# craftsangjae/instance-segmentation-road-project

Measured on AMD Instinct MI355X. Metric: images/sec at 1024x1024 (MaskLab inference hot path, full forward), higher is better.
Workload: dtype f32; 1 GPU; resnext50_full_b8_1024; per_gpu_batch=8, global_batch=8, height=1024, width=1024, parallelism=dp1, hipgraph=False, inputs=resident in HBM, weights=random init (cls logits x8 so NMS / mask head run at full load)

## Files before the change

### include/masklab_hip.h

```cpp
#ifndef MASKLAB_HIP_H
#define MASKLAB_HIP_H

#include <stdint.h>

#ifdef __cplusplus
extern "C" {
#endif

#define ML_OK 0
#define ML_E_BADARG (-1)
#define ML_E_LAUNCH (-2)
#define ML_E_NOGPU  (-3)

enum { ML_ACT_NONE = 0, ML_ACT_RELU = 1, ML_ACT_RELU6 = 2, ML_ACT_SIGMOID = 3 };
enum { ML_MATH_F32 = 0, ML_MATH_F16 = 1, ML_MATH_F16S = 2, ML_MATH_F32X3 = 3 };

#define ML_ABI_VERSION 7
int ml_version(void);
const char *ml_last_error(void);
int ml_device_check(void);

typedef struct ml_conv2d_desc {
    const float *in;
    const float *wgt;
    const float *bias;
    const float *residual;
    float *out;
    int32_t B, H, W;
    int32_t in_cstride, in_coff;
    int32_t span;
    int32_t span_pad;
    int32_t cpp_shift;
    int32_t Ho, Wo;
    int32_t KH, KW, stride, dil, pad_t, pad_l;
    int32_t cout;
    int32_t n_pad;
    int32_t out_cstride, out_coff;
    int32_t res_cstride, res_coff;
    int32_t act;
    int32_t group_cin_step;
    int32_t shuffle2x2;
    int32_t tile;
    int32_t math;
    int32_t out_f16;
    int64_t out_bstride;
    const int32_t *live;
    int32_t live_period;
    int32_t reserved1;
    double *gn_partials;
} ml_conv2d_desc;

int ml_conv2d_f32(const ml_conv2d_desc *d, void *stream);

#define ML_CONV_MAX_PROBLEMS 12
int64_t ml_conv2d_workspace_bytes(void);
int ml_conv2d_multi_f32(const ml_conv2d_desc *descs, int32_t n, void *workspace, int64_t workspace_bytes,
                        void *stream);
int ml_conv2d_ntile(int32_t cout, int32_t tile);
int ml_conv2d_launch_ntile(const ml_conv2d_desc *descs, int32_t n, int32_t has_workspace);
int ml_conv2d_launch_mtile(const ml_conv2d_desc *descs, int32_t n, int32_t has_workspace);
int ml_conv2d_uses_pipe(const ml_conv2d_desc *d);
int ml_conv2d_launch_splits(const ml_conv2d_desc *descs, int32_t n, int64_t workspace_bytes, int32_t *splits);
int ml_conv2d_wino_eligible(const ml_conv2d_desc *d);
int64_t ml_conv2d_gn_min_launch_tiles(void);

int ml_gconv3x3_f32(const float *in, const float *wgt, const float *bias, float *out,
                    int32_t B, int32_t H, int32_t W, int32_t C, int32_t c, int32_t Ho, int32_t Wo,
                    int32_t stride, int32_t pad_t, int32_t pad_l, int32_t act, void *stream);

int ml_gconv3x3_f16(const void *in, const float *wgt, const float *bias, void *out,
                    int32_t B, int32_t H, int32_t W, int32_t C, int32_t c, int32_t Ho, int32_t Wo,
                    int32_t stride, int32_t pad_t, int32_t pad_l, int32_t act, void *stream);

int ml_maxpool3x3s2_f16(const void *in, void *out, int32_t B, int32_t H, int32_t W, int32_t C,
                        int32_t Ho, int32_t Wo, int32_t pad_t, int32_t pad_l, void *stream);
int ml_subsample2_f16(const void *in, void *out, int32_t B, int32_t H, int32_t W, int32_t C, void *stream);
int ml_cast_f16_to_f32(const void *in, float *out, int64_t n, void *stream);
int ml_cast_f32_to_f16(const float *in, void *out, int64_t n, void *stream);
int ml_resize_bilinear_ac_f16(const void *in, const void *add, void *out,
                              int32_t B, int32_t H, int32_t W, int32_t C, int32_t in_cstride, int32_t in_coff,
                              int32_t Ho, int32_t Wo, int32_t add_cstride, int32_t add_coff,
                              int32_t out_cstride, int32_t out_coff, void *stream);
int ml_dwconv3x3_f16(const void *in, const float *wgt, const float *bias, void *out,
                     int32_t B, int32_t H, int32_t W, int32_t C, int32_t in_cstride, int32_t in_coff,
                     int32_t out_cstride, int32_t out_coff, int32_t Ho, int32_t Wo,
                     int32_t stride, int32_t dil, int32_t pad_t, int32_t pad_l, int32_t act, void *stream);
int ml_global_mean_f16(const void *in, void *out, int32_t B, int32_t HW, int32_t C, void *stream);

int ml_stem7x7s2_pool_f16(const float *image, const void *wgt_h, const float *bias, void *out, int32_t B, int32_t H,
                          int32_t W, int32_t Hp, int32_t Wp, void *stream);
int ml_stem7x7s2_pool_f32(const float *image, const float *wgt, const float *bias, float *out, int32_t B, int32_t H,
                          int32_t W, int32_t Hp, int32_t Wp, void *stream);
int ml_stem7x7s2_pool_x3(const float *image, const void *wgt_x3, const float *bias, float *out, int32_t B, int32_t H,
                         int32_t W, int32_t Hp, int32_t Wp, void *stream);

typedef struct ml_deconv_out_problem {
    const float *x, *wd, *bd, *wo_table, *bo;
    float *out;
    int64_t M;
    int32_t hw, w, rois_per_image, reserved0;
    int64_t out_image_stride, out_base;
    const int32_t *live;
} ml_deconv_out_problem;
int ml_deconv2x2_out1x1_f32(const ml_deconv_out_problem *probs, int32_t nprob, int32_t K, int32_t c_mid, int32_t ncls,
                            int32_t cp, int32_t act_mid, int32_t act_out, void *stream);
int ml_deconv2x2_out1x1_f16(const ml_deconv_out_problem *probs, int32_t nprob, int32_t K, int32_t c_mid, int32_t ncls,
                            int32_t cp, int32_t act_mid, int32_t act_out, void *stream);

int ml_dwconv3x3_f32(const float *in, const float *wgt, const float *bias, float *out,
                     int32_t B, int32_t H, int32_t W, int32_t C,
                     int32_t in_cstride, int32_t in_coff, int32_t out_cstride, int32_t out_coff,
                     int32_t Ho, int32_t Wo, int32_t stride, int32_t dil,
                     int32_t pad_t, int32_t pad_l, int32_t act, void *stream);

int ml_maxpool3x3s2_f32(const float *in, float *out, int32_t B, int32_t H, int32_t W, int32_t C,
                        int32_t Ho, int32_t Wo, int32_t pad_t, int32_t pad_l, void *stream);

int ml_preprocess_f32(const void *in, int32_t is_u8, float *out, int64_t npix, int32_t out_c,
                      int32_t flip, const float *mean, const float *div, const float *shift,
                      void *stream);

int64_t ml_groupnorm_workspace_bytes(int32_t N, int32_t G);
int ml_groupnorm_chunk_f32(const float *x, float *y, const float *gamma, const float *beta,
                           int32_t N, int64_t HWC, int32_t C, int32_t G, float eps, int32_t relu,
                           int32_t out_cstride, int32_t out_coff,
                           void *workspace, void *stream);
int ml_groupnorm_chunk_f16(const void *x, void *y, const float *gamma, const float *beta,
                           int32_t N, int64_t HWC, int32_t C, int32_t G, float eps, int32_t relu,
                           int32_t out_cstride, int32_t out_coff, void *workspace, void *stream);

typedef struct ml_gn_desc {
    const float *x;
    float *y;
    const float *gamma, *beta;
    int64_t HWC;
    int32_t N, C, G, relu;
    int32_t out_cstride, out_coff;
    float eps;
    int32_t dtype;
    const int32_t *live;
    int32_t live_period, reserved;
    const double *partials;
    int32_t n_partials, reserved2;
} ml_gn_desc;
#define ML_GN_MAX_PROBLEMS 8
int ml_groupnorm_multi_f32(const ml_gn_desc *descs, int32_t n, void *workspace, int64_t workspace_bytes, void *stream);
// ... 237 lines not shown
```

### instance-segmentation-road-project_amd/csrc/conv_wino.hip

```cpp
#include "common.h"

namespace {

constexpr int WMAXP = ML_CONV_MAX_PROBLEMS;
constexpr int WT = 64;
constexpr int WN = 64;
constexpr int WK = 8;
constexpr int WCHUNK = WK * 32 * 16;
constexpr int WSTEP = 4 * 32 * 16;
constexpr int NSLOT_P = 3;
constexpr int SLOT_P = WT * 16 * 8;
constexpr int NSLOT_W = 4;
constexpr int SLOT_W = 2 * WSTEP;
constexpr int RING_W = NSLOT_P * SLOT_P;
constexpr int LDS_BYTES = (RING_W + NSLOT_W * SLOT_W) * 4;
static_assert(LDS_BYTES == 160 * 1024, "the two rings fill the CU's LDS");
#ifndef WINO_EXP
#define WINO_EXP 0
#endif
constexpr unsigned OOB = 0x80000000u;
constexpr long long SPAN_MAX = 0x7fffff00ll;

struct WProblem {
    ml_conv2d_desc d;
// ... 13 lines not shown
#endif
}

__device__ __forceinline__ void bt_d_b_op(int k, const float d[16], float t[16], float v[16]) {
    if (k < 16) {
        const int j = k >> 2;
        switch (k & 3) {
            case 0: t[0 * 4 + j] = d[0 * 4 + j] - d[2 * 4 + j]; break;
            case 1: t[1 * 4 + j] = d[1 * 4 + j] + d[2 * 4 + j]; break;
            case 2: t[2 * 4 + j] = d[2 * 4 + j] - d[1 * 4 + j]; break;
            default: t[3 * 4 + j] = d[1 * 4 + j] - d[3 * 4 + j]; break;
        }
    } else {
        const int i = (k - 16) >> 2;
        switch (k & 3) {
            case 0: v[i * 4 + 0] = t[i * 4 + 0] - t[i * 4 + 2]; break;
            case 1: v[i * 4 + 1] = t[i * 4 + 1] + t[i * 4 + 2]; break;
            case 2: v[i * 4 + 2] = t[i * 4 + 2] - t[i * 4 + 1]; break;
            default: v[i * 4 + 3] = t[i * 4 + 1] - t[i * 4 + 3]; break;
        }
    }
}

__global__ void __launch_bounds__(512, 1) conv_wino_kernel(const WArgs args) {
    extern __shared__ __align__(16) float lds[];

    int pi = 0;
    while (pi + 1 < args.n && (int)blockIdx.x >= args.start[pi + 1]) ++pi;
    const WProblem &P = args.p[pi];
    const ml_conv2d_desc &p = P.d;
    const int b = (int)blockIdx.x - args.start[pi];
    const int g = b / (8 * P.NB), rr = b - g * 8 * P.NB;
    const int nt2 = rr >> 3;
    const int mt = g * 8 + (rr & 7);
    if (mt >= P.MB) return;
    if (p.live) {
        const int lv = max(1, *p.live), tpi0 = P.TH * P.TW;
        const int b0 = mt * WT / tpi0, b1 = min(mt * WT + WT, P.T) - 1;
        bool any = false;
        for (int bi = b0; bi <= b1 / tpi0 && !any; ++bi) any = bi % p.live_period < lv;
        if (!any) return;
    }

    const int tid = threadIdx.x, lane = tid & 63;
    const int wave = __builtin_amdgcn_readfirstlane(tid >> 6);
    const int tg = wave & 3, h = wave >> 2;
    const int r = lane & 15, kq = lane >> 4;
    const int tpi = P.TH * P.TW;

    const int gt0 = mt * WT;
    long long base_pix;
    {
        const int bi = gt0 / tpi, rem = gt0 - bi * tpi, ty = rem / P.TW;
        base_pix = ((long long)bi * p.H + max(2 * ty - 1, 0)) * p.W;
    }
    const size_t cstride = (size_t)p.in_cstride;
    const float *pin = p.in + p.in_coff + (size_t)base_pix * cstride;
    int voff_p[4];
    {
        const int rt = (lane >> 1) & 15;
        const int quad = (lane & 1) ^ ((rt >> 2) & 1);
        const int gt = gt0 + (wave >> 1) * 16 + rt;
        int bi = 0, ty = 0, tx = 0;
        if (gt < P.T) {
            bi = gt / tpi;
            const int rem = gt - bi * tpi;
            ty = rem / P.TW;
            tx = rem - ty * P.TW;
        }
#pragma unroll
        for (int i = 0; i < 4; ++i) {
            const int px = 8 * (wave & 1) + 2 * i + (lane >> 5);
            const int y = 2 * ty - 1 + (px >> 2), x = 2 * tx - 1 + (px & 3);
            voff_p[i] = (int)OOB;
            if (gt < P.T && y >= 0 && y < p.H && x >= 0 && x < p.W)
                voff_p[i] = (int)((((long long)bi * p.H + y) * p.W + x - base_pix) * (long long)cstride * 4) + quad * 16;
        }
    }
    const int voff_w = ((wave & 3) * 512 + r * 16 + kq * 4) * 4;
    const float *wsrc = p.wgt + (size_t)(2 * nt2 + (wave >> 2)) * P.nchunks * WCHUNK;
    float *dst_p = lds + (wave >> 1) * 2048 + (wave & 1) * 1024;
    float *dst_w = lds + RING_W + (wave >> 2) * WSTEP + (wave & 3) * 512;
    const int nch = P.nchunks, nsteps = 2 * P.nchunks;

    auto rsrc_p = [&](int j) __attribute__((always_inline)) {
        const bool real = j < nch && !(WINO_EXP & 1);
        return __builtin_amdgcn_make_buffer_rsrc((void *)(pin + j * 8), 0, real ? (int)OOB : 0, 0x00020000);
    };
    auto rsrc_w = [&](int s) __attribute__((always_inline)) {
        const bool real = s < nsteps && !(WINO_EXP & 2);
        return __builtin_amdgcn_make_buffer_rsrc((void *)(wsrc + (size_t)s * WSTEP), 0, real ? WSTEP * 4 : 0, 0x00020000);
    };

    f32x4 acc[2][16];
#pragma unroll
    for (int t = 0; t < 2; ++t)
#pragma unroll
        for (int q = 0; q < 16; ++q) acc[t][q] = f32x4{0.f, 0.f, 0.f, 0.f};

    const float *pa_lane0 = lds + tg * 2048 + r * 8 + 4 * ((r >> 2) & 1) + kq;
    const float *pa_lane1 = lds + tg * 2048 + r * 8 + 4 * (((r >> 2) & 1) ^ 1) + kq;
    const float *pb_lane = lds + RING_W + h * WSTEP + kq * 512 + r * 4;
    struct Ops {
        float d[16], t[16], v[16];
        f32x4 b[2][4];
    };
    auto read_ops = [&](const float *pa, const float *pb, Ops &o) __attribute__((always_inline)) {
#pragma unroll
        for (int t = 0; t < 2; ++t)
#pragma unroll
            for (int pq = 0; pq < 4; ++pq) o.b[t][pq] = *reinterpret_cast<const f32x4 *>(pb + t * 256 + pq * 64);
#pragma unroll
        for (int px = 0; px < 16; ++px) o.d[px] = pa[px * 128];
    };

    auto step = [&](const Ops &cur, Ops &nxt, const float *pa, const float *pb, const int ndma, auto dma) __attribute__((always_inline)) {
#if WINO_EXP == 4
#pragma unroll
        for (int q = 0; q < ndma; ++q) dma(q);
        __builtin_amdgcn_sched_barrier(0);
#endif
#pragma unroll
        for (int m = 0; m < 32; ++m) {
            const int t = m >> 4, pq = (m >> 2) & 3, e = m & 3;
            acc[t][4 * pq + e] =
                __builtin_amdgcn_mfma_f32_16x16x4f32(cur.v[4 * pq + e], cur.b[t][pq][e], acc[t][4 * pq + e], 0, 0, 0);
            if (m == 3) {
                __builtin_amdgcn_sched_barrier(0);
                read_ops(pa, pb, nxt);
                __builtin_amdgcn_sched_barrier(0);
            }
#if WINO_EXP != 4
            if (m % 6 == 5 && m / 6 < ndma) {
                __builtin_amdgcn_sched_barrier(0);
                dma(m / 6);
                __builtin_amdgcn_sched_barrier(0);
            }
#endif
            if (m >= 16) {
                bt_d_b_op(2 * (m - 16), nxt.d, nxt.t, nxt.v);
                bt_d_b_op(2 * (m - 16) + 1, nxt.d, nxt.t, nxt.v);
                __builtin_amdgcn_sched_barrier(0);
            }
        }
    };

    {
        const __amdgpu_buffer_rsrc_t rp0 = rsrc_p(0), rp1 = rsrc_p(1), rw0 = rsrc_w(0), rw1 = rsrc_w(1), rw2 = rsrc_w(2);
#pragma unroll
        for (int i = 0; i < 4; ++i) dma16(rp0, dst_p + i * 256, voff_p[i]);
        dma16(rw0, dst_w, voff_w);
        dma16(rw0, dst_w + 256, voff_w + 1024);
#pragma unroll
        for (int i = 0; i < 4; ++i) dma16(rp1, dst_p + SLOT_P + i * 256, voff_p[i]);
        dma16(rw1, dst_w + SLOT_W, voff_w);
        dma16(rw1, dst_w + SLOT_W + 256, voff_w + 1024);
        dma16(rw2, dst_w + 2 * SLOT_W, voff_w);
        dma16(rw2, dst_w + 2 * SLOT_W + 256, voff_w + 1024);
    }
    Ops oa, ob;
    asm volatile("s_waitcnt vmcnt(8)" ::: "memory");
    __builtin_amdgcn_s_barrier();
    read_ops(pa_lane0, pb_lane, oa);
#pragma unroll
    for (int k = 0; k < 32; ++k) bt_d_b_op(k, oa.d, oa.t, oa.v);

    int ps0 = 0, ps1 = SLOT_P, ps2 = 2 * SLOT_P;
    for (int j = 0; j < nch; ++j) {
        const int w0 = (2 * j) & 3;
        const int wa = ((w0 ^ 2) + 1) * SLOT_W, wb = w0 * SLOT_W;
        asm volatile("s_waitcnt vmcnt(0) lgkmcnt(0)" ::: "memory");
        __builtin_amdgcn_s_barrier();
        const __amdgpu_buffer_rsrc_t rp = rsrc_p(j + 2), rwa = rsrc_w(2 * j + 3), rwb = rsrc_w(2 * j + 4);
        auto dma = [&](int q) __attribute__((always_inline)) {
            if (q < 4) dma16(rp, dst_p + ps2 + q * 256, voff_p[q]);
            else if (q < 6) dma16(rwa, dst_w + wa + (q - 4) * 256, voff_w + (q - 4) * 1024);
            else dma16(rwb, dst_w + wb + (q - 6) * 256, voff_w + (q - 6) * 1024);
        };
        step(oa, ob, pa_lane1 + ps0, pb_lane + (w0 + 1) * SLOT_W, 5, dma);
        step(ob, oa, pa_lane0 + ps1, pb_lane + (w0 ^ 2) * SLOT_W, 3, [&](int q) __attribute__((always_inline)) { dma(q + 5); });
        const int ps = ps0;
        ps0 = ps1;
        ps1 = ps2;
        ps2 = ps;
    }
    asm volatile("s_waitcnt vmcnt(0)" ::: "memory");

    const int nt = 2 * nt2 + h;
    const bool gn = p.gn_partials != nullptr;
    double gs[2] = {0.0, 0.0}, gq[2] = {0.0, 0.0};
    long long f0 = 0;
    if (gn) {
        const int bi = gt0 / tpi, rem = gt0 - bi * tpi, ty = rem / P.TW, tx = rem - ty * P.TW;
        f0 = ((long long)(bi * p.Ho + 2 * ty) * p.Wo + 2 * tx) >> 7;
    }
    const float lo = 0.f, hi = (p.act == ML_ACT_RELU6) ? 6.f : 3.402823466e38f;
    const bool clampv = p.act == ML_ACT_RELU || p.act == ML_ACT_RELU6;
#pragma unroll
    for (int i = 0; i < 4; ++i) {
        const int gt = gt0 + tg * 16 + kq * 4 + i;
        if (gt >= P.T) continue;
        const int bi = gt / tpi, rem = gt - bi * tpi;
        const int ty = rem / P.TW, tx = rem - ty * P.TW;
        const int oy = 2 * ty, ox = 2 * tx;
        const bool y1 = oy + 1 < p.Ho, x1 = ox + 1 < p.Wo;
        const size_t img = p.out_bstride ? (size_t)bi * (size_t)p.out_bstride : (size_t)bi * p.Ho * p.Wo * p.out_cstride;
        const size_t pix0 = (size_t)oy * p.Wo + ox;
#pragma unroll
        for (int t = 0; t < 2; ++t) {
            const int n = nt * 32 + 16 * t + r;
            if (n >= p.cout) continue;
            float m[16];
#pragma unroll
            for (int q = 0; q < 16; ++q) m[q] = acc[t][q][i];
            float u[8];
#pragma unroll
            for (int j = 0; j < 4; ++j) {
                u[j] = m[0 * 4 + j] + m[1 * 4 + j] + m[2 * 4 + j];
                u[4 + j] = m[1 * 4 + j] - m[2 * 4 + j] - m[3 * 4 + j];
            }
            float yv[4];
#pragma unroll
            for (int a = 0; a < 2; ++a) {
                yv[2 * a] = u[4 * a + 0] + u[4 * a + 1] + u[4 * a + 2];
                yv[2 * a + 1] = u[4 * a + 1] - u[4 * a + 2] - u[4 * a + 3];
            }
            const float bv = p.bias ? p.bias[n] : 0.f;
            float *o = p.out + img + p.out_coff + n;
#pragma unroll
            for (int a = 0; a < 2; ++a)
#pragma unroll
                for (int c2 = 0; c2 < 2; ++c2) {
                    if ((a && !y1) || (c2 && !x1)) continue;
                    float val = yv[2 * a + c2] + bv;
                    if (clampv) val = __builtin_amdgcn_fmed3f(val, lo, hi);
                    else if (p.act != ML_ACT_NONE) val = ml_apply_act(val, p.act);
                    o[(pix0 + (size_t)a * p.Wo + c2) * p.out_cstride] = val;
                    if (gn) {
                        const long long m_flat = ((long long)(bi * p.Ho + oy + a) * p.Wo + ox + c2);
                        const int f = (m_flat >> 7) != f0;
                        gs[f] += (double)val;
                        gq[f] += (double)val * (double)val;
                    }
                }
        }
    }
    if (gn) {
        double *lds_gn = reinterpret_cast<double *>(lds);
        __syncthreads();
#pragma unroll
        for (int o = 32; o > 0; o >>= 1) {
#pragma unroll
            for (int f = 0; f < 2; ++f) {
                gs[f] += __shfl_down(gs[f], o, 64);
                gq[f] += __shfl_down(gq[f], o, 64);
            }
        }
        if (lane == 0) {
            lds_gn[wave * 4 + 0] = gs[0]; lds_gn[wave * 4 + 1] = gq[0];
            lds_gn[wave * 4 + 2] = gs[1]; lds_gn[wave * 4 + 3] = gq[1];
        }
        __syncthreads();
        if (tid < 4) {
            const int hh = tid >> 1, ff = tid & 1;
            const int gt1 = gt0 + WT - 1;
            const int bi = gt1 / tpi, rem = gt1 - bi * tpi, ty = rem / P.TW, tx = rem - ty * P.TW;
            const long long f1 = ((long long)(bi * p.Ho + 2 * ty + 1) * p.Wo + 2 * tx + 1) >> 7;
            const long long ft = ff ? f1 : f0;
            const int slot = 2 * nt2 + hh;
            double s = 0.0, q = 0.0;
            for (int w = 0; w < 4; ++w) { s += lds_gn[(hh * 4 + w) * 4 + 2 * ff]; q += lds_gn[(hh * 4 + w) * 4 + 2 * ff + 1]; }
            p.gn_partials[2 * (ft * 4 + slot)] = s;
            p.gn_partials[2 * (ft * 4 + slot) + 1] = q;
        }
    }
}

}

extern "C" int ml_conv2d_wino_eligible(const ml_conv2d_desc *d) {
    if (!d) return 0;
    return d->math == ML_MATH_F32 && d->KH == 3 && d->KW == 3 && d->stride == 1 && d->dil == 1 && d->pad_t == 1 &&
           d->pad_l == 1 && d->Ho == d->H && d->Wo == d->W && d->cpp_shift == 30 && d->group_cin_step == 0 &&
           !d->shuffle2x2 && !d->residual && !d->out_f16 && d->span % 32 == 0 && d->span_pad == d->span &&
           d->cout <= 128 && d->n_pad == 128;
}

int ml_conv2d_wino_gn_ok(const ml_conv2d_desc &d) {
    if (d.Ho % 2 || d.Wo % 2 || d.cout != 128 || d.out_bstride || d.act == ML_ACT_SIGMOID) return 0;
    const long long TH = d.Ho / 2, TW = d.Wo / 2;
    return (64 % TW == 0 || TW % 64 == 0) && (TH * TW) % 64 == 0;
}

int ml_conv2d_wino_launch(const ml_conv2d_desc *descs, int n, hipStream_t s) {
    ML_REQUIRE(n >= 1 && n <= WMAXP, "conv2d (winograd): need 1..%d problems", WMAXP);
    WArgs args;
    args.n = n;
    long long start = 0;
    for (int i = 0; i < n; ++i) {
        const ml_conv2d_desc &d = descs[i];
        ML_REQUIRE(ml_conv2d_wino_eligible(&d),
                   "conv2d: tile = 6 (Winograd F(2x2,3x3)) needs ML_MATH_F32, a 3x3 stride-1 undilated 'same' conv, no "
                   "groups / shuffle / residual / half output, span %% 32 == 0 and n_pad == 128");
        ML_REQUIRE(((d.in_cstride | d.in_coff) & 3) == 0 && ml_aligned16(d.in) && ml_aligned16(d.wgt),
                   "conv2d (winograd): 16-byte aligned input channels and weights");
        if (d.gn_partials)
            ML_REQUIRE(ml_conv2d_wino_gn_ok(d) && !d.live, "conv2d (winograd): gn_partials needs even Ho / Wo, Wo / 2 dividing or a "
                                                "multiple of 64, (Ho / 2) (Wo / 2) %% 64 == 0, cout = 128, dense output");
        WProblem &P = args.p[i];
        P.d = d;
        P.TH = (d.Ho + 1) / 2;
        P.TW = (d.Wo + 1) / 2;
        const long long T = (long long)d.B * P.TH * P.TW;
        ML_REQUIRE(T < (1ll << 30), "conv2d (winograd): too many tiles");
        P.T = (int)T;
        P.MB = (int)((T + WT - 1) / WT);
        P.NB = d.n_pad / WN;
        P.nchunks = d.span_pad / WK;
        const long long span = (2ll * (WT / P.TW + 2) + 2) * d.W * d.in_cstride * 4;
        ML_REQUIRE(span <= SPAN_MAX, "conv2d (winograd): a block's input rows exceed 2 GiB (W x in_cstride too large)");
        args.start[i] = (int)start;
        start += (long long)(P.MB + 7) / 8 * 8 * P.NB;
        ML_REQUIRE(start < (1ll << 31), "conv2d (winograd): grid too large");
    }
    args.start[n] = (int)start;
    long long tiles128 = 0;
    bool any_gn = false;
    for (int i = 0; i < n; ++i) {
        tiles128 += ((long long)descs[i].B * descs[i].Ho * descs[i].Wo + 127) / 128 * (descs[i].n_pad / 128);
        any_gn = any_gn || descs[i].gn_partials != nullptr;
    }
    ML_REQUIRE(!any_gn || tiles128 >= ml_conv2d_gn_min_launch_tiles(),
               "conv2d (winograd): gn_partials needs a launch of ml_conv2d_gn_min_launch_tiles() tiles of 128 x 128");
    static std::atomic<unsigned long long> lds_ok{0};
    if (int rc = ml_ensure_dynamic_lds(reinterpret_cast<const void *>(conv_wino_kernel), LDS_BYTES, lds_ok, "conv2d (winograd)"))
        return rc;
    hipLaunchKernelGGL(conv_wino_kernel, dim3((unsigned)start), dim3(512), LDS_BYTES, s, args);
    ML_CHECK_LAUNCH("conv2d (winograd)");
    return ML_OK;
}
```

### instance-segmentation-road-project_amd/masklab_hip/_lib.py

```python
import ctypes as C
import os

_HERE = os.path.dirname(os.path.abspath(__file__))
LIB_PATH = os.path.join(_HERE, "libmasklab_hip.so")

ABI_VERSION = 7
ACT_NONE, ACT_RELU, ACT_RELU6, ACT_SIGMOID = 0, 1, 2, 3
ACT_BY_NAME = {None: ACT_NONE, "linear": ACT_NONE, "relu": ACT_RELU, "relu6": ACT_RELU6,
               "sigmoid": ACT_SIGMOID}


class ConvDesc(C.Structure):
    _fields_ = [
        ("in_", C.c_void_p), ("wgt", C.c_void_p), ("bias", C.c_void_p),
        ("residual", C.c_void_p), ("out", C.c_void_p),
        ("B", C.c_int32), ("H", C.c_int32), ("W", C.c_int32),
        ("in_cstride", C.c_int32), ("in_coff", C.c_int32),
        ("span", C.c_int32), ("span_pad", C.c_int32), ("cpp_shift", C.c_int32),
        ("Ho", C.c_int32), ("Wo", C.c_int32),
        ("KH", C.c_int32), ("KW", C.c_int32), ("stride", C.c_int32), ("dil", C.c_int32),
        ("pad_t", C.c_int32), ("pad_l", C.c_int32),
        ("cout", C.c_int32), ("n_pad", C.c_int32),
        ("out_cstride", C.c_int32), ("out_coff", C.c_int32),
        ("res_cstride", C.c_int32), ("res_coff", C.c_int32),
        ("act", C.c_int32), ("group_cin_step", C.c_int32), ("shuffle2x2", C.c_int32),
        ("tile", C.c_int32), ("math", C.c_int32), ("out_f16", C.c_int32),
        ("out_bstride", C.c_int64),
        ("live", C.c_void_p), ("live_period", C.c_int32), ("reserved1", C.c_int32),
        ("gn_partials", C.c_void_p),
    ]


class GnDesc(C.Structure):
    _fields_ = [("x", C.c_void_p), ("y", C.c_void_p), ("gamma", C.c_void_p), ("beta", C.c_void_p),
                ("HWC", C.c_int64), ("N", C.c_int32), ("C", C.c_int32), ("G", C.c_int32), ("relu", C.c_int32),
                ("out_cstride", C.c_int32), ("out_coff", C.c_int32), ("eps", C.c_float), ("dtype", C.c_int32),
                ("live", C.c_void_p), ("live_period", C.c_int32), ("reserved", C.c_int32),
                ("partials", C.c_void_p), ("n_partials", C.c_int32), ("reserved2", C.c_int32)]


class DeconvOutProblem(C.Structure):
    _fields_ = [("x", C.c_void_p), ("wd", C.c_void_p), ("bd", C.c_void_p), ("wo_table", C.c_void_p),
                ("bo", C.c_void_p), ("out", C.c_void_p), ("M", C.c_int64), ("hw", C.c_int32), ("w", C.c_int32),
                ("rois_per_image", C.c_int32), ("reserved0", C.c_int32), ("out_image_stride", C.c_int64),
                ("out_base", C.c_int64), ("live", C.c_void_p)]


class SeDesc(C.Structure):
    _fields_ = [("x", C.c_void_p), ("out", C.c_void_p), ("w1", C.c_void_p), ("w2", C.c_void_p),
                ("B", C.c_int32), ("HW", C.c_int32), ("C", C.c_int32), ("Hd", C.c_int32),
                ("live", C.c_void_p), ("live_period", C.c_int32), ("reserved", C.c_int32), ("ws_offset", C.c_int64)]


class SeResidualDesc(C.Structure):
    _fields_ = [("x", C.c_void_p), ("shortcut", C.c_void_p), ("w1", C.c_void_p), ("b1", C.c_void_p),
                ("w2", C.c_void_p), ("b2", C.c_void_p), ("scale", C.c_void_p), ("shift", C.c_void_p),
                ("out_act", C.c_void_p), ("out_y", C.c_void_p),
                ("B", C.c_int32), ("HW", C.c_int32), ("C", C.c_int32), ("Hd", C.c_int32),
                ("mode", C.c_int32), ("reserved", C.c_int32)]


class SeBottleneckDesc(C.Structure):
    _fields_ = [("c3", C.c_void_p), ("residual", C.c_void_p), ("w1", C.c_void_p), ("b1", C.c_void_p),
                ("w2", C.c_void_p), ("b2", C.c_void_p), ("out", C.c_void_p),
                ("B", C.c_int32), ("HW", C.c_int32), ("C", C.c_int32), ("Hd", C.c_int32)]


SE_RES_GATE, SE_RES_BN_RELU = 0, 1
GN_MAX_PROBLEMS = 8
SE_MAX_PROBLEMS = 8
DECONV_OUT_MAX_PROBLEMS = 4
_i32, _i64, _f32, _vp = C.c_int32, C.c_int64, C.c_float, C.c_void_p

SIGNATURES = {
    "ml_version": (C.c_int, []),
    "ml_last_error": (C.c_char_p, []),
    "ml_device_check": (C.c_int, []),
    "ml_conv2d_f32": (C.c_int, [C.POINTER(ConvDesc), _vp]),
    "ml_conv2d_ntile": (C.c_int, [_i32, _i32]),
    "ml_conv2d_uses_pipe": (C.c_int, [C.POINTER(ConvDesc)]),
    "ml_conv2d_launch_ntile": (C.c_int, [C.POINTER(ConvDesc), _i32, _i32]),
    "ml_conv2d_launch_mtile": (C.c_int, [C.POINTER(ConvDesc), _i32, _i32]),
    "ml_conv2d_launch_splits": (C.c_int, [C.POINTER(ConvDesc), _i32, _i64, C.POINTER(C.c_int32)]),
    "ml_conv2d_wino_eligible": (C.c_int, [C.POINTER(ConvDesc)]),
    "ml_conv2d_gn_min_launch_tiles": (_i64, []),
    "ml_conv2d_workspace_bytes": (_i64, []),
    "ml_conv2d_multi_f32": (C.c_int, [C.POINTER(ConvDesc), _i32, _vp, _i64, _vp]),
    "ml_deconv2x2_out1x1_f32": (C.c_int, [C.POINTER(DeconvOutProblem), _i32, _i32, _i32, _i32, _i32, _i32, _i32, _vp]),
    "ml_gconv3x3_f32": (C.c_int, [_vp, _vp, _vp, _vp] + [_i32] * 11 + [_vp]),
    "ml_gconv3x3_f16": (C.c_int, [_vp, _vp, _vp, _vp] + [_i32] * 11 + [_vp]),
    "ml_maxpool3x3s2_f16": (C.c_int, [_vp, _vp] + [_i32] * 8 + [_vp]),
    "ml_stem7x7s2_pool_f16": (C.c_int, [_vp, _vp, _vp, _vp] + [_i32] * 5 + [_vp]),
    "ml_stem7x7s2_pool_f32": (C.c_int, [_vp, _vp, _vp, _vp] + [_i32] * 5 + [_vp]),
    "ml_stem7x7s2_pool_x3": (C.c_int, [_vp, _vp, _vp, _vp] + [_i32] * 5 + [_vp]),
    "ml_subsample2_f16": (C.c_int, [_vp, _vp] + [_i32] * 4 + [_vp]),
    "ml_cast_f16_to_f32": (C.c_int, [_vp, _vp, _i64, _vp]),
    "ml_cast_f32_to_f16": (C.c_int, [_vp, _vp, _i64, _vp]),
    "ml_resize_bilinear_ac_f16": (C.c_int, [_vp, _vp, _vp] + [_i32] * 12 + [_vp]),
    "ml_dwconv3x3_f16": (C.c_int, [_vp, _vp, _vp, _vp] + [_i32] * 15 + [_vp]),
    "ml_global_mean_f16": (C.c_int, [_vp, _vp, _i32, _i32, _i32, _vp]),
    "ml_groupnorm_chunk_f16": (C.c_int, [_vp, _vp, _vp, _vp, _i32, _i64, _i32, _i32, _f32, _i32, _i32, _i32, _vp, _vp]),
    "ml_roi_crop_resize_f16": (C.c_int, [_vp, _vp, _i32, _i32, _vp, _vp, _vp, _vp] + [_i32] * 10 + [_f32, _f32, _i32, _i32, _vp, _vp]),
    "ml_deconv2x2_out1x1_f16": (C.c_int, [C.POINTER(DeconvOutProblem), _i32, _i32, _i32, _i32, _i32, _i32, _i32, _vp]),
    "ml_dwconv3x3_f32": (C.c_int, [_vp, _vp, _vp, _vp] + [_i32] * 15 + [_vp]),
    "ml_maxpool3x3s2_f32": (C.c_int, [_vp, _vp] + [_i32] * 8 + [_vp]),
    "ml_preprocess_f32": (C.c_int, [_vp, _i32, _vp, _i64, _i32, _i32, C.POINTER(C.c_float), C.POINTER(C.c_float),
                                    C.POINTER(C.c_float), _vp]),
    "ml_groupnorm_workspace_bytes": (_i64, [_i32, _i32]),
    "ml_groupnorm_multi_f32": (C.c_int, [C.POINTER(GnDesc), _i32, _vp, _i64, _vp]),
    "ml_groupnorm_chunk_f32": (C.c_int, [_vp, _vp, _vp, _vp, _i32, _i64, _i32, _i32, _f32, _i32, _i32, _i32, _vp, _vp]),
    "ml_resize_bilinear_ac_f32": (C.c_int, [_vp, _vp, _vp] + [_i32] * 12 + [_vp]),
    "ml_global_mean_f32": (C.c_int, [_vp, _vp, _i32, _i32, _i32, _vp]),
    "ml_scale_channels_f32": (C.c_int, [_vp, _vp, _i32, _i32, _i32, _vp]),
    "ml_squeeze_excite_workspace_bytes": (_i64, [_i32, _i32, _i32]),
    "ml_squeeze_excite_f32": (C.c_int, [C.POINTER(SeDesc), _i32, _vp, _i64, _vp]),
    "ml_squeeze_excite_f16": (C.c_int, [C.POINTER(SeDesc), _i32, _vp, _i64, _vp]),
    "ml_se_residual_workspace_bytes": (_i64, [_i32, _i32, _i32]),
    "ml_se_residual_f32": (C.c_int, [C.POINTER(SeResidualDesc), _vp, _i64, _vp]),
    "ml_se_bottleneck_workspace_bytes": (_i64, [_i32, _i32, _i32]),
    "ml_se_bottleneck_f32": (C.c_int, [C.POINTER(SeBottleneckDesc), _vp, _i64, _vp]),
    "ml_se_bottleneck_f16": (C.c_int, [C.POINTER(SeBottleneckDesc), _vp, _i64, _vp]),
    "ml_conv1x1_dual_f32": (C.c_int, [_vp] * 5 + [_i32] * 7 + [_vp]),
    "ml_conv1x1_dual_f16": (C.c_int, [_vp] * 5 + [_i32] * 7 + [_vp]),
    "ml_restore_boxes_f32": (C.c_int, [_vp, _vp, _vp, _i32, _i32, _vp]),
    "ml_detection_workspace_bytes": (_i64, [_i32, _i32, _i32, _i32]),
    "ml_detection_proposal_f32": (C.c_int, [_vp, _vp, _vp, _vp, _vp, _vp, _i32, _i32, _i32, _f32, _f32, _f32, _i32, _vp, _vp]),
    "ml_mask_distribute_i32": (C.c_int, [_vp, _i32, _i32, _vp, _vp, _vp, _vp, _i32, _i32, _i32, _f32, _vp]),
    "ml_roi_crop_resize_f32": (C.c_int, [_vp, _vp, _i32, _i32, _vp, _vp, _vp, _vp] + [_i32] * 10 + [_f32, _f32, _i32, _i32, _vp, _vp]),
    "ml_mold_levels_f32": (C.c_int, [_vp, _vp, _i32, _i32, _i32, _i64, C.POINTER(C.c_int32), _vp]),
    "ml_mold_levels_dev_f32": (C.c_int, [_vp, _vp, _i32, _i32, _i32, _i64, _vp, _vp]),
    "ml_add_f32": (C.c_int, [_vp, _vp, _i64, _vp]),
    "ml_add_f16": (C.c_int, [_vp, _vp, _i64, _vp]),
    "ml_fill_f32": (C.c_int, [_vp, _f32, _i64, _vp]),
    "ml_resize_image_ac": (C.c_int, [_vp, _i32, _vp, _vp, _f32] + [_i32] * 6 + [_vp]),
    "ml_trim_instances_f32": (C.c_int, [_vp] * 5 + [_i32] * 5 + [_vp]),
    "ml_upsample_boxes_i32": (C.c_int, [_vp, _vp, _i64, _f32, _f32, _vp]),
    "ml_threshold_i32": (C.c_int, [_vp, _vp, _f32, _i64, _vp]),
    "ml_semantic_smoothing_f32": (C.c_int, [_vp, _vp, _vp] + [_i32] * 4 + [_vp, _vp, _vp]),
    "ml_crop_pad_mask_f32": (C.c_int, [_vp, _vp, _vp, _vp] + [_i32] * 6 + [_vp]),
    "ml_nonzero_bbox_i32": (C.c_int, [_vp] + [_i32] * 5 + [_vp, _vp]),
    "ml_instance_summary_workspace_bytes": (_i64, [_i32, _i32]),
    "ml_instance_summary_f32": (C.c_int, [_vp, _i32, _i32, _vp, _vp] + [_i32] * 4 + [_f32, _f32, _vp, _vp]),
    "ml_instance_summary_rois_f32": (C.c_int, [_vp, _i32, _i32, _vp, _vp, _vp] + [_i32] * 6 + [_f32, _f32, _vp, _vp]),
    "ml_draw_boxes_u8": (C.c_int, [_vp, _vp, _vp] + [_i32] * 4 + [_vp]),
    "ml_draw_instance_u8": (C.c_int, [_vp, _vp, _vp, _vp, _vp, _i32, _f32] + [_i32] * 4 + [_vp]),
    "ml_draw_segmentation_u8": (C.c_int, [_vp, _vp, _i32, _vp, _vp, _i32, _f32] + [_i32] * 3 + [_vp]),
    "ml_serving_visualize_u8": (C.c_int, [_vp] * 7 + [_i32, _f32, _vp, _i32, _f32] + [_i32] * 6 + [_vp]),
    "ml_jpeg_encode_capacity": (_i64, [_i32, _i32]),
    "ml_jpeg_encode_workspace_bytes": (_i64, [_i32, _i32, _i32]),
    "ml_jpeg_encode_u8": (C.c_int, [_vp] + [_i32] * 4 + [_vp, _i64, _vp, _vp, _vp]),
    "ml_jpeg_decode_info": (C.c_int, [_vp, _i64, _vp]),
    "ml_jpeg_decode_packed_bytes": (_i64, [_vp, _i64]),
    "ml_jpeg_decode_entropy": (_i64, [_vp, _i64, _vp, _i64]),
    "ml_jpeg_decode_workspace_bytes": (_i64, [_i32] * 4),
    "ml_jpeg_decode_u8": (C.c_int, [_vp, _vp] + [_i32] * 4 + [_vp, _vp, _vp]),
    "ml_jpeg_decode_reference_host": (C.c_int, [_vp, _vp] + [_i32] * 4 + [_vp, _vp]),
    "ml_jpeg_entropy_geometry": (C.c_int, [_vp]),
    "ml_jpeg_entropy_plan_bytes": (_i64, []),
    "ml_jpeg_entropy_plan": (C.c_int, [_vp, _i64, _vp]),
    "ml_jpeg_entropy_workspace_bytes": (_i64, [_vp, _i32]),
    "ml_jpeg_entropy_device": (C.c_int, [_vp, _vp, _vp, _i32, _vp, _vp, _vp, _vp, _vp]),
    "ml_jpeg_entropy_reference_host": (C.c_int, [_vp, _i64, _vp, _vp, _i64, _vp, _vp]),
    "ml_eval_mask_area": (C.c_int, [_vp] + [_i32] * 4 + [_vp, _vp]),
    "ml_eval_mask_pairs": (C.c_int, [_vp] * 5 + [_i32] * 8 + [_vp, _vp]),
    "ml_eval_semantic_counts": (C.c_int, [_vp, _vp] + [_i32] * 4 + [_vp, _vp]),
    "ml_eval_class_binary_iou": (C.c_int, [_vp, _i32, _vp, _i32, _i32, _i64, _i32, _f32, _vp, _vp, _vp]),
    "ml_eval_detection_metric_f32": (C.c_int, [_vp, _vp, _i32, _i32, _i32, _vp, _vp]),
# ... 55 lines not shown
```

### instance-segmentation-road-project_amd/masklab_hip/ops.py

```python
import ctypes as C
import threading

import numpy as np
import torch

from . import _lib
from .packing import PackedConv, pack_winograd, resolve_padding

import weakref

_ws_cache = {}
_ws_retired = []
_graph_owners = weakref.WeakSet()


def graph_owner_registered(model):
    _graph_owners.add(model)


def graph_owner_released(model):
    _graph_owners.discard(model)
    if not len(_graph_owners):
        _ws_retired.clear()

# ... 174 lines not shown
        d.out_cstride, d.out_coff, d.out_bstride = out.shape[3], out_coff, 0
    x3 = CONV_MATH == "f32x3" and not half_in
    d.in_, d.wgt, d.bias = x.data_ptr(), (dc.wgt_h if half_in else (dc.wgt_x3 if x3 else dc.wgt)).data_ptr(), \
        (dc.bias.data_ptr() if dc.bias is not None else None)
    if residual is not None:
        _require_dev(residual, "residual")
        if tuple(residual.shape[:3]) != (B, Ho, Wo):
            raise ValueError("conv2d: residual spatial shape mismatch")
        d.residual, d.res_cstride, d.res_coff = residual.data_ptr(), residual.shape[3], 0
    d.B, d.H, d.W = B, H, W
    d.in_cstride, d.in_coff = Cbuf, in_coff
    d.span, d.span_pad, d.cpp_shift = p.span, (dc.span_pad_h if half_in else p.span_pad), p.cpp_shift
    d.Ho, d.Wo = Ho, Wo
    d.KH, d.KW, d.stride, d.dil, d.pad_t, d.pad_l = p.KH, p.KW, stride, dilation, pt, pl
    d.cout, d.n_pad = p.cout, p.n_pad
    d.act, d.group_cin_step, d.shuffle2x2, d.tile = act, p.group_cin_step, p.shuffle2x2, p.tile
    if gn_partials is not None:
        _require_dev(gn_partials, "gn_partials")
        if gn_partials.dtype != torch.float64 or gn_partials.numel() < 8 * ((B * Ho * Wo + 127) // 128):
            raise ValueError("conv2d: gn_partials must be a float64 tensor of 4 x 2 values per 128-row tile")
        if d.out_coff % 4 or d.out_cstride % 4:
            raise ValueError("conv2d: gn_partials needs a destination slice aligned to 4 channels")
        d.gn_partials = gn_partials.data_ptr()
    if live is not None:
        lv, period = live
        _require_dev(lv, "live")
        d.live, d.live_period = lv.data_ptr(), int(period)
    if half_in:
        d.math, d.out_f16 = 2, int(odt == torch.float16)
    else:
        d.math, d.out_f16 = _MATH_CODE[CONV_MATH], int(odt == torch.float16)
        if d.out_f16 and d.math != 1:
            raise ValueError("conv2d: a half output from fp32 input needs the fp16 MFMA mode (set_conv_math('f16s'))")
    M = B * Ho * Wo
    real_cin = p.span if p.cpp_shift == 30 else 3
    es_in, es_out = x.element_size(), (2 if odt == torch.float16 else 4)
    nbytes = (es_in * B * H * W * real_cin * (1 if not p.group_cin_step else p.n_pad // 32) + es_out * M * p.cout +
              es_in * p.cout * p.k_real + (es_out * M * p.cout if residual is not None else 0))
    shape = f"M={M} N={p.cout} K={p.KH * p.KW * d.span_pad} k{p.kh_real}x{p.kw_real} s{stride} d{dilation} HxW={H}x{W}"
    return d, ret, (2.0 * M * p.cout * p.k_real, nbytes, shape)


def _conv_kernel_name(descs, n, p, half):
    lib = _lib.load()
    which = lib.ml_conv2d_uses_pipe(descs) if n == 1 else 0
    if which:
        return "conv1x1_h256_h" if which == 2 else (
            "conv1x1_pipe_h" if half else ("conv1x1_pipe_x3" if CONV_MATH == "f32x3" else "conv1x1_pipe"))
    bn = lib.ml_conv2d_launch_ntile(descs, n, 1) or lib.ml_conv2d_ntile(p.cout, p.tile)
    bm = lib.ml_conv2d_launch_mtile(descs, n, 1) or 128
    return "conv_mfma_%dx%d%s%s" % (bm, bn, "_grouped" if p.group_cin_step else "",
                                     "_h" if half else {"f32": "", "f32x3": "_x3"}.get(CONV_MATH, "_f16"))


def _launch_conv(descs, problems, flops, nbytes, shapes, multi):
    lib = _lib.load()
    n = len(problems)
    x, dc = problems[0]
    wino = _wino_select(descs, n, problems)
    label = ("multi x%d" % n if multi else shapes[0]) + (" wino direct_flop=%.0f" % flops if wino else "")
    if wino:
        flops = sum(_wino_flops(descs[i]) for i in range(n))
    ws = workspace(int(lib.ml_conv2d_workspace_bytes()), x.device, "conv")
    if LAUNCH_LOG is not None:
        sp = (C.c_int32 * n)()
        _lib.check(lib.ml_conv2d_launch_splits(descs, n, ws.numel(), sp), "ml_conv2d_launch_splits")
        LAUNCH_LOG.append((" | ".join(shapes) if multi else label, tuple(int(v) for v in sp)))
    name = None
    if PROFILE is not None:
        name = "conv_wino_f32" if wino else _conv_kernel_name(descs, n, dc.p, x.dtype == torch.float16)
    with _Prof(name, flops, nbytes, label) as prof:
        if prof.on and name == "conv1x1_h256_h":
            d = descs[0]
            M, N, K = d.B * d.Ho * d.Wo, d.cout, d.span
            prof.rec["staged_bytes"] = float(-(-M // 256) * (N // 256) * 2 * 256 * K * 2)
        _lib.check(lib.ml_conv2d_multi_f32(descs, n, _ptr(ws), ws.numel(), _stream()), "ml_conv2d_multi_f32")


def _wino_select(descs, n, problems):
    if CONV_MATH != "f32":
        return False
    lib = _lib.load()
    for i, (x, dc) in enumerate(problems):
        if x.dtype != torch.float32 or dc.p.tile != 0 or not lib.ml_conv2d_wino_eligible(C.byref(descs[i])):
            return False
    for i, (x, dc) in enumerate(problems):
        descs[i].tile = 6
        descs[i].wgt = dc.wgt_wino.data_ptr()
    return True


def _wino_flops(d):
    return 2.0 * d.B * ((d.Ho + 1) // 2) * ((d.Wo + 1) // 2) * 16 * d.span * d.cout


def _wino_gn_ok(out_shape):
    _, Ho, Wo = out_shape
    if Ho % 2 or Wo % 2:
        return False
    th, tw = Ho // 2, Wo // 2
    return (64 % tw == 0 or tw % 64 == 0) and (th * tw) % 64 == 0


def gn_fusable(out_shape, C_out, groups, dc, launch_tiles, dtype):
    B, Ho, Wo = out_shape
    hw = Ho * Wo
    p = dc.p
    math_ok = (CONV_MATH in ("f32", "f32x3") and dtype == torch.float32) or (CONV_MATH == "f16s" and dtype == torch.float16)
    ok = (math_ok and C_out == 128 and p.cout == 128 and p.n_pad == 128 and
          not p.shuffle2x2 and not p.group_cin_step and hw % 128 == 0 and hw % groups == 0 and (hw // groups) % 128 == 0 and
          launch_tiles >= _gn_min_launch_tiles())
    if ok and CONV_MATH == "f32" and p.KH == 3 and p.KW == 3 and p.cpp_shift == 30 and p.tile == 0:
        ok = _wino_gn_ok(out_shape)
    return 4 * ((hw // groups) // 128) if ok else 0


_GN_MIN_TILES = None


def _gn_min_launch_tiles():
    global _GN_MIN_TILES
    if _GN_MIN_TILES is None:
        _GN_MIN_TILES = int(_lib.load().ml_conv2d_gn_min_launch_tiles())
    return _GN_MIN_TILES


def conv2d(x, dc: DeviceConv, stride=1, padding="same", dilation=1, act=_lib.ACT_NONE,
           residual=None, out=None, out_coff=0, in_coff=0, out_view=None, out_dtype=None, gn_partials=None):
    if x.dtype == torch.float16 and stride == 2 and dc.p.kh_real == 1 and dc.p.kw_real == 1:
        x, stride = subsample2_h(x), 1
    d, ret, (flops, nbytes, shape) = _conv_desc(x, dc, stride, padding, dilation, act, residual, out, out_coff,
                                                in_coff, out_view, out_dtype, gn_partials=gn_partials)
    _launch_conv((_lib.ConvDesc * 1)(d), [(x, dc)], flops, nbytes, [shape], multi=False)
    return ret


def conv2d_multi(problems):
    n = len(problems)
    if n == 0:
        return []
    if n > 12:
        return conv2d_multi(problems[:12]) + conv2d_multi(problems[12:])
    arr = (_lib.ConvDesc * n)()
    rets, flops, nbytes, shapes = [], 0.0, 0.0, []
    for i, pr in enumerate(problems):
        pr = dict(pr)
        d, ret, (f, nb, shape) = _conv_desc(pr.pop("x"), pr.pop("dc"), **pr)
        arr[i] = d
        rets.append(ret)
        flops += f
        nbytes += nb
        shapes.append(shape)
    _launch_conv(arr, [(pr["x"], pr["dc"]) for pr in problems], flops, nbytes, shapes, multi=True)
    return rets


def deconv2x2_out1x1_multi(problems, ncls, act_mid, act_out):
    lib = _lib.load()
    n = len(problems)
    if n == 0:
        return
    if n > _lib.DECONV_OUT_MAX_PROBLEMS:
        deconv2x2_out1x1_multi(problems[:_lib.DECONV_OUT_MAX_PROBLEMS], ncls, act_mid, act_out)
        deconv2x2_out1x1_multi(problems[_lib.DECONV_OUT_MAX_PROBLEMS:], ncls, act_mid, act_out)
        return
    arr = (_lib.DeconvOutProblem * n)()
    flops = nbytes = 0.0
    K = cmid = cp = None
    for i, pr in enumerate(problems):
        x, dc, out = pr["x"], pr["dc"], pr["out"]
# ... 1426 lines not shown
```

### instance-segmentation-road-project_amd/masklab_hip/packing.py

```python
import math
from dataclasses import dataclass, field

import numpy as np

NO_PIX_SPAN = 30


def same_pads(size, k, stride, dilation=1):
    out = -(-size // stride)
    k_eff = (k - 1) * dilation + 1
    total = max((out - 1) * stride + k_eff - size, 0)
    return out, total // 2, total - total // 2


def resolve_padding(H, W, kh, kw, stride, dilation, padding):
    if padding == "same":
        Ho, pt, _ = same_pads(H, kh, stride, dilation)
        Wo, pl, _ = same_pads(W, kw, stride, dilation)
        return Ho, Wo, pt, pl
    if padding == "valid":
        pt = pb = pl = pr = 0
    else:
        (pt, pb), (pl, pr) = padding
    Ho = (H + pt + pb - ((kh - 1) * dilation + 1)) // stride + 1
# ... 94 lines not shown
    g = n // c
    m = n % c
    win0 = (n // 32) * 32
    for i in range(c):
        cin_idx = g * c + i
        w[n, :, :, cin_idx - win0] = np.transpose(dw_kernel[:, :, cin_idx, m], (2, 0, 1))
    w2d, n_pad = _pad_rows(w.reshape(filters, kh * kw * 32), filters, 3)
    assert n_pad == filters or filters % 32
    return PackedConv(wgt=w2d, bias=None if bias is None else np.ascontiguousarray(bias, np.float32),
                      KH=kh, KW=kw, span=32, span_pad=32, cout=filters, n_pad=n_pad, group_cin_step=32,
                      tile=3, cin_buffer=filters, kh_real=kh, kw_real=kw, k_real=kh * kw * c)


def pack_grouped_mfma4(dw_kernel, groups):
    kh, kw, filters, c = dw_kernel.shape
    assert (kh, kw) == (3, 3) and filters == groups * c
    k = dw_kernel.reshape(3, 3, groups, c, c)
    return np.ascontiguousarray(np.transpose(k, (2, 4, 0, 1, 3)).reshape(filters, 9, c), np.float32)


def grouped_dw_to_dense(dw_kernel, groups):
    kh, kw, filters, c = dw_kernel.shape
    wg = np.zeros((kh, kw, c, filters), dw_kernel.dtype)
    for g in range(groups):
        for i in range(c):
            wg[:, :, i, g * c:(g + 1) * c] = dw_kernel[:, :, g * c + i, :]
    return wg


def pack_transpose2x2(kernel, bias=None, tile=0):
    assert kernel.shape[:2] == (2, 2)
    _, _, cout, cin = kernel.shape
    if cin % 4:
        raise ValueError("transposed conv needs cin % 4 == 0")
    span_pad = -(-cin // 32) * 32
    w = np.zeros((4 * cout, span_pad), np.float32)
    w[:, :cin] = kernel.reshape(4 * cout, cin)
    w2d, n_pad = _pad_rows(w, 4 * cout, tile)
    return PackedConv(wgt=w2d, bias=None if bias is None else np.ascontiguousarray(bias, np.float32),
                      KH=1, KW=1, span=cin, span_pad=span_pad, cout=4 * cout, n_pad=n_pad, shuffle2x2=1,
                      tile=tile, cin_buffer=cin, k_real=cin)


def pack_out1x1_table(kernel, bias=None):
    assert kernel.shape[:2] == (1, 1)
    cmid, ncls = int(kernel.shape[2]), int(kernel.shape[3])
    if cmid % 32 or ncls > 32:
        raise ValueError("fused mask-head tail needs C_mid % 32 == 0 and at most 32 classes")
    cp = 1
    while cp < ncls:
        cp *= 2
    t, e, h = np.meshgrid(np.arange(cmid // 32), np.arange(16), np.arange(2), indexing="ij")
    ch = 32 * t + (e & 3) + 8 * (e >> 2) + 4 * h
    table = np.zeros((cmid // 32, 16, 2, cp), np.float32)
    table[..., :ncls] = kernel[0, 0][ch]
    b = np.zeros((cp,), np.float32)
    if bias is not None:
        b[:ncls] = bias
    return np.ascontiguousarray(table), b, cp


def pack_depthwise(dw_kernel):
    kh, kw, C, mult = dw_kernel.shape
    assert (kh, kw, mult) == (3, 3, 1)
    return np.ascontiguousarray(dw_kernel.reshape(9, C), np.float32)


WINO_G = np.array([[1.0, 0.0, 0.0], [0.5, 0.5, 0.5], [0.5, -0.5, 0.5], [0.0, 0.0, 1.0]])
WINO_BT = np.array([[1.0, 0.0, -1.0, 0.0], [0.0, 1.0, 1.0, 0.0], [0.0, -1.0, 1.0, 0.0], [0.0, 1.0, 0.0, -1.0]])
WINO_AT = np.array([[1.0, 1.0, 1.0, 0.0], [0.0, 1.0, -1.0, -1.0]])


def winograd_transform(g):
    return np.einsum("ai,...ij,bj->...ab", WINO_G, np.asarray(g, np.float64), WINO_G)


def pack_winograd(packed: PackedConv):
    p = packed
    if (p.KH, p.KW) != (3, 3) or p.cpp_shift != NO_PIX_SPAN or p.group_cin_step or p.shuffle2x2 or p.n_pad % 32 or p.span_pad % 8:
        raise ValueError("winograd packing needs a dense 3x3 conv (n_pad % 32 == 0)")
    g = p.wgt.reshape(p.n_pad, 3, 3, p.span_pad).transpose(0, 3, 1, 2)
    u = winograd_transform(g).reshape(p.n_pad, p.span_pad, 16).astype(np.float32)
    u = u.reshape(p.n_pad // 32, 32, p.span_pad // 8, 8, 16).transpose(0, 2, 3, 1, 4)
    return np.ascontiguousarray(u)
```

Baseline: 423.8 images/sec.

## Route narrow-cout 3x3 convs through Winograd kernel with dead-half skipping

Lets 3x3 convs whose padded output width is 32/64/96 (with cout not exactly 32 or 64) use the Winograd F(2,3) kernel. Their weights are zero-padded to 128 output rows and the descriptor is rewritten to n_pad=128. The launch grid now sizes its N blocks from cout instead of n_pad. Waves whose 32-column half lies past cout skip all math and only keep issuing the input DMAs and barriers in lockstep, with s_sleep between them. This trades the previous direct-conv path for Winograd arithmetic on these layers, at the cost of idle waves still occupying LDS and barrier slots.

```diff
diff --git a/include/masklab_hip.h b/include/masklab_hip.h
--- a/include/masklab_hip.h
+++ b/include/masklab_hip.h
@@ -62,6 +62,7 @@
 int ml_conv2d_uses_pipe(const ml_conv2d_desc *d);
 int ml_conv2d_launch_splits(const ml_conv2d_desc *descs, int32_t n, int64_t workspace_bytes, int32_t *splits);
 int ml_conv2d_wino_eligible(const ml_conv2d_desc *d);
+int ml_conv2d_wino_narrow(const ml_conv2d_desc *d);
 int64_t ml_conv2d_gn_min_launch_tiles(void);
 
 int ml_gconv3x3_f32(const float *in, const float *wgt, const float *bias, float *out,
diff --git a/instance-segmentation-road-project_amd/csrc/conv_wino.hip b/instance-segmentation-road-project_amd/csrc/conv_wino.hip
--- a/instance-segmentation-road-project_amd/csrc/conv_wino.hip
+++ b/instance-segmentation-road-project_amd/csrc/conv_wino.hip
@@ -119,13 +119,14 @@
     float *dst_p = lds + (wave >> 1) * 2048 + (wave & 1) * 1024;
     float *dst_w = lds + RING_W + (wave >> 2) * WSTEP + (wave & 3) * 512;
     const int nch = P.nchunks, nsteps = 2 * P.nchunks;
+    const bool dead = (2 * nt2 + h) * 32 >= p.cout;
 
     auto rsrc_p = [&](int j) __attribute__((always_inline)) {
         const bool real = j < nch && !(WINO_EXP & 1);
         return __builtin_amdgcn_make_buffer_rsrc((void *)(pin + j * 8), 0, real ? (int)OOB : 0, 0x00020000);
     };
     auto rsrc_w = [&](int s) __attribute__((always_inline)) {
-        const bool real = s < nsteps && !(WINO_EXP & 2);
+        const bool real = s < nsteps && !dead && !(WINO_EXP & 2);
         return __builtin_amdgcn_make_buffer_rsrc((void *)(wsrc + (size_t)s * WSTEP), 0, real ? WSTEP * 4 : 0, 0x00020000);
     };
 
@@ -195,9 +196,31 @@
         dma16(rw2, dst_w + 2 * SLOT_W, voff_w);
         dma16(rw2, dst_w + 2 * SLOT_W + 256, voff_w + 1024);
     }
-    Ops oa, ob;
     asm volatile("s_waitcnt vmcnt(8)" ::: "memory");
     __builtin_amdgcn_s_barrier();
+
+    if (dead) {
+        int ps2 = 2 * SLOT_P;
+        for (int j = 0; j < nch; ++j) {
+            const int w0 = (2 * j) & 3;
+            const int wa = ((w0 ^ 2) + 1) * SLOT_W, wb = w0 * SLOT_W;
+            asm volatile("s_waitcnt vmcnt(0) lgkmcnt(0)" ::: "memory");
+            __builtin_amdgcn_s_barrier();
+            const __amdgpu_buffer_rsrc_t rp = rsrc_p(j + 2), rwa = rsrc_w(2 * j + 3), rwb = rsrc_w(2 * j + 4);
+#pragma unroll
+            for (int q = 0; q < 8; ++q) {
+                if (q < 4) dma16(rp, dst_p + ps2 + q * 256, voff_p[q]);
+                else if (q < 6) dma16(rwa, dst_w + wa + (q - 4) * 256, voff_w + (q - 4) * 1024);
+                else dma16(rwb, dst_w + wb + (q - 6) * 256, voff_w + (q - 6) * 1024);
+                __builtin_amdgcn_s_sleep(3);
+            }
+            ps2 = ps2 == 2 * SLOT_P ? 0 : ps2 + SLOT_P;
+        }
+        asm volatile("s_waitcnt vmcnt(0)" ::: "memory");
+        return;
+    }
+
+    Ops oa, ob;
     read_ops(pa_lane0, pb_lane, oa);
 #pragma unroll
     for (int k = 0; k < 32; ++k) bt_d_b_op(k, oa.d, oa.t, oa.v);
@@ -321,6 +344,15 @@
            d->pad_l == 1 && d->Ho == d->H && d->Wo == d->W && d->cpp_shift == 30 && d->group_cin_step == 0 &&
            !d->shuffle2x2 && !d->residual && !d->out_f16 && d->span % 32 == 0 && d->span_pad == d->span &&
            d->cout <= 128 && d->n_pad == 128;
+}
+
+extern "C" int ml_conv2d_wino_narrow(const ml_conv2d_desc *d) {
+    if (!d || d->live || d->gn_partials) return 0;
+    if (d->n_pad != 32 && d->n_pad != 64 && d->n_pad != 96) return 0;
+    if (d->cout < 1 || d->cout > d->n_pad || d->cout == 32 || d->cout == 64) return 0;
+    ml_conv2d_desc w = *d;
+    w.n_pad = 128;
+    return ml_conv2d_wino_eligible(&w);
 }
 
 int ml_conv2d_wino_gn_ok(const ml_conv2d_desc &d) {
@@ -352,7 +384,7 @@
         ML_REQUIRE(T < (1ll << 30), "conv2d (winograd): too many tiles");
         P.T = (int)T;
         P.MB = (int)((T + WT - 1) / WT);
-        P.NB = d.n_pad / WN;
+        P.NB = (d.cout + WN - 1) / WN;
         P.nchunks = d.span_pad / WK;
         const long long span = (2ll * (WT / P.TW + 2) + 2) * d.W * d.in_cstride * 4;
         ML_REQUIRE(span <= SPAN_MAX, "conv2d (winograd): a block's input rows exceed 2 GiB (W x in_cstride too large)");
diff --git a/instance-segmentation-road-project_amd/masklab_hip/_lib.py b/instance-segmentation-road-project_amd/masklab_hip/_lib.py
--- a/instance-segmentation-road-project_amd/masklab_hip/_lib.py
+++ b/instance-segmentation-road-project_amd/masklab_hip/_lib.py
@@ -83,6 +83,7 @@
     "ml_conv2d_launch_mtile": (C.c_int, [C.POINTER(ConvDesc), _i32, _i32]),
     "ml_conv2d_launch_splits": (C.c_int, [C.POINTER(ConvDesc), _i32, _i64, C.POINTER(C.c_int32)]),
     "ml_conv2d_wino_eligible": (C.c_int, [C.POINTER(ConvDesc)]),
+    "ml_conv2d_wino_narrow": (C.c_int, [C.POINTER(ConvDesc)]),
     "ml_conv2d_gn_min_launch_tiles": (_i64, []),
     "ml_conv2d_workspace_bytes": (_i64, []),
     "ml_conv2d_multi_f32": (C.c_int, [C.POINTER(ConvDesc), _i32, _vp, _i64, _vp]),
diff --git a/instance-segmentation-road-project_amd/masklab_hip/ops.py b/instance-segmentation-road-project_amd/masklab_hip/ops.py
--- a/instance-segmentation-road-project_amd/masklab_hip/ops.py
+++ b/instance-segmentation-road-project_amd/masklab_hip/ops.py
@@ -280,10 +280,12 @@
         return False
     lib = _lib.load()
     for i, (x, dc) in enumerate(problems):
-        if x.dtype != torch.float32 or dc.p.tile != 0 or not lib.ml_conv2d_wino_eligible(C.byref(descs[i])):
+        if x.dtype != torch.float32 or dc.p.tile != 0:
+            return False
+        if not (lib.ml_conv2d_wino_eligible(C.byref(descs[i])) or lib.ml_conv2d_wino_narrow(C.byref(descs[i]))):
             return False
     for i, (x, dc) in enumerate(problems):
-        descs[i].tile = 6
+        descs[i].tile, descs[i].n_pad = 6, 128
         descs[i].wgt = dc.wgt_wino.data_ptr()
     return True
 
diff --git a/instance-segmentation-road-project_amd/masklab_hip/packing.py b/instance-segmentation-road-project_amd/masklab_hip/packing.py
--- a/instance-segmentation-road-project_amd/masklab_hip/packing.py
+++ b/instance-segmentation-road-project_amd/masklab_hip/packing.py
@@ -200,4 +200,6 @@
     g = p.wgt.reshape(p.n_pad, 3, 3, p.span_pad).transpose(0, 3, 1, 2)
     u = winograd_transform(g).reshape(p.n_pad, p.span_pad, 16).astype(np.float32)
     u = u.reshape(p.n_pad // 32, 32, p.span_pad // 8, 8, 16).transpose(0, 2, 3, 1, 4)
+    if u.shape[0] < 4:
+        u = np.concatenate([u, np.zeros((4 - u.shape[0],) + u.shape[1:], np.float32)])
     return np.ascontiguousarray(u)
```

Measured after the change: 428.8 images/sec (median of 6 runs). 1.2% higher.
